# nanoporetech/medaka

Measured on NVIDIA H100. Metric: pileup positions/sec (consensus inference), higher is better.
Workload: dtype f32

## Files before the change

medaka_b200/csrc/gru_wg.cu:

```cuda
#include "common.cuh"
#include "ptx.cuh"
#include "rec_common.cuh"

namespace mdk {

constexpr int RW_THREADS = 256;
constexpr int RW_ABLK = (H / 8) * 64 * 16;
constexpr int RW_XBLK = 2 * 64 * 16;

template <int NT, bool FUSE_X, int OUT>
struct RwCfg {
    static constexpr int N = NT * RT_N;
    static constexpr bool HL = NT == 1;
    static constexpr int ROWS = HL ? 2 * N : N;
    static constexpr int PLANES = HL ? 1 : 2;
    static constexpr int KG = ROWS * 16 + 16;
    static constexpr int HPLANE = (H / 8) * KG;
    static constexpr int XPLANE = 2 * KG;
    static constexpr int HLO = HL ? N * 16 : HPLANE;
    static constexpr int XLO = HL ? N * 16 : XPLANE;
    static constexpr int RED = (RW_THREADS / 32) * NCLS * N;
    static constexpr int wlo_off = 0;
    static constexpr int wxlo_off = wlo_off + 6 * RW_ABLK;
    static constexpr int h_off = wxlo_off + (FUSE_X ? 6 * RW_XBLK : 0);
    static constexpr int x_off = h_off + 2 * PLANES * HPLANE;
    static constexpr int red_off = x_off + (FUSE_X ? 2 * PLANES * XPLANE : 0);
    static constexpr int total = red_off + (OUT == OUT_LOGITS ? 2 * RED * 4 : 0);
    static_assert(total <= 227 * 1024, "smem budget");
};

__device__ __forceinline__ uint32_t ld_u32(const __half *p) { return *reinterpret_cast<const uint32_t *>(p); }

template <int NT, bool FUSE_X, int OUT>
__global__ void __launch_bounds__(RW_THREADS, 1)
rec_tc_kernel(const float *__restrict__ gi, RecX xin, const __half *__restrict__ w_hh, const float *__restrict__ b_hn,
              void *__restrict__ h_out, int64_t B, int64_t T, const float *__restrict__ lin_w,
              float *__restrict__ plog) {
    using L = RwCfg<NT, FUSE_X, OUT>;
    constexpr int N = L::N, NA = N / 2;
    constexpr int NACC = L::ROWS / 2;
    constexpr int NX = FUSE_X ? NACC : NA;
    using MMA = Wgmma<N>;
    using MMA_H = Wgmma<L::ROWS>;
    constexpr bool LOGITS = OUT == OUT_LOGITS;
    extern __shared__ __align__(128) uint8_t smem[];
    const int tid = threadIdx.x, wg = tid >> 7, warp = (tid >> 5) & 3, lane = tid & 31;
    const int gq = lane >> 2, cq = lane & 3;
    const int dir = blockIdx.y;
    const int64_t ntiles = (B + RT_N - 1) / RT_N;
    const int64_t wtile0 = (int64_t)blockIdx.x * NT;
    const int j0 = wg * 64 + warp * 16 + gq;
    const uint32_t sbase = smem_u32(smem);

    for (int i = tid; i < (L::total - L::h_off) / 16; i += RW_THREADS)
        reinterpret_cast<int4 *>(smem + L::h_off)[i] = make_int4(0, 0, 0, 0);
    for (int i = tid; i < 3 * H * (H / 8); i += RW_THREADS) {
        const int kg = i & 15, r = (i >> 4) & (H - 1), gate = i >> 11;
        const uint4 v = *reinterpret_cast<const uint4 *>(w_hh + ((((size_t)dir * 2 + 1) * 3 + gate) * H + r) * H + kg * 8);
        *reinterpret_cast<uint4 *>(smem + L::wlo_off + (gate * 2 + (r >> 6)) * RW_ABLK + kg * 1024 + (r & 63) * 16) = v;
    }
    if (FUSE_X) {
        for (int i = tid; i < 3 * H * 2; i += RW_THREADS) {
            const int kg = i & 1, r = (i >> 1) & (H - 1), gate = i >> 8;
            const uint4 v = *reinterpret_cast<const uint4 *>(xin.w_x + ((((size_t)dir * 2 + 1) * 3 + gate) * H + r) * 16 + kg * 8);
            *reinterpret_cast<uint4 *>(smem + L::wxlo_off + (gate * 2 + (r >> 6)) * RW_XBLK + kg * 1024 + (r & 63) * 16) = v;
        }
    }
    float wlin[2][NCLS];
    if (LOGITS) {
#pragma unroll
        for (int hb = 0; hb < 2; ++hb)
#pragma unroll
            for (int c = 0; c < NCLS; ++c) wlin[hb][c] = lin_w[c * H2 + dir * H + j0 + 8 * hb];
    }
    uint32_t whi[3][H / 16][4];
#pragma unroll
    for (int gate = 0; gate < 3; ++gate)
#pragma unroll
        for (int ks = 0; ks < H / 16; ++ks) {
            const __half *w = w_hh + ((((size_t)dir * 2) * 3 + gate) * H + j0) * H + ks * 16 + 2 * cq;
            whi[gate][ks][0] = ld_u32(w);
            whi[gate][ks][1] = ld_u32(w + 8 * H);
            whi[gate][ks][2] = ld_u32(w + 8);
            whi[gate][ks][3] = ld_u32(w + 8 * H + 8);
        }
    uint32_t wxhi[3][4];
    float bx[3][2] = {};
    if (FUSE_X) {
#pragma unroll
        for (int gate = 0; gate < 3; ++gate) {
            const __half *w = xin.w_x + ((((size_t)dir * 2) * 3 + gate) * H + j0) * 16 + 2 * cq;
            wxhi[gate][0] = ld_u32(w);
            wxhi[gate][1] = ld_u32(w + 8 * 16);
            wxhi[gate][2] = ld_u32(w + 8);
            wxhi[gate][3] = ld_u32(w + 8 * 16 + 8);
            bx[gate][0] = xin.bias[dir * G3 + gate * H + j0];
            bx[gate][1] = xin.bias[dir * G3 + gate * H + j0 + 8];
        }
    }
    const float bhn[2] = {b_hn[dir * H + j0], b_hn[dir * H + j0 + 8]};

    float ar[NACC], az[NACC], an[NACC], axn[NX], hp[NA];
#pragma unroll
    for (int k = 0; k < NA; ++k) hp[k] = 0.f;
    const float *gi_thr = FUSE_X ? nullptr
                                 : gi + wtile0 * T * GI_TS_FLOATS + ((dir * 3 * 4 + (cq >> 1)) * H + j0) * 4 + 2 * (cq & 1);
    auto load_pre = [&](int64_t t) {
#pragma unroll
        for (int i = 0; i < N / 8; ++i)
#pragma unroll
            for (int hb = 0; hb < 2; ++hb) {
                float2 v[3] = {make_float2(0.f, 0.f), make_float2(0.f, 0.f), make_float2(0.f, 0.f)};
                if (FUSE_X) {
#pragma unroll
                    for (int gate = 0; gate < 3; ++gate) v[gate] = make_float2(bx[gate][hb], bx[gate][hb]);
                } else if (i < 2 || wtile0 + (i >> 1) < ntiles) {
                    const float *p = gi_thr + ((i >> 1) * T + t) * GI_TS_FLOATS + (2 * (i & 1) * H + 8 * hb) * 4;
#pragma unroll
                    for (int gate = 0; gate < 3; ++gate) v[gate] = __ldcs(reinterpret_cast<const float2 *>(p + gate * 16 * H));
                }
                const int k = 4 * i + 2 * hb;
                ar[k] = v[0].x; ar[k + 1] = v[0].y;
                az[k] = v[1].x; az[k + 1] = v[1].y;
                axn[k] = v[2].x; axn[k + 1] = v[2].y;
                an[k] = bhn[hb]; an[k + 1] = bhn[hb];
            }
        if constexpr (L::HL) {
#pragma unroll
            for (int k = NA; k < NACC; ++k) {
                ar[k] = 0.f; az[k] = 0.f; an[k] = 0.f;
                if constexpr (FUSE_X) axn[k] = 0.f;
            }
        }
    };
    const int xF = FUSE_X ? xin.F : 1;
    const float *xsrc[NT];
    int xoff[NT];
    float xreg[NT];
#pragma unroll
    for (int m = 0; m < NT; ++m) {
        const int q = tid + RW_THREADS * m, xn = q / xF, xf = q - xn * xF;
        const bool own = FUSE_X && q < N * xF;
        xoff[m] = own ? (xf >> 3) * L::KG + xn * 16 + (xf & 7) * 2 : -1;
        xsrc[m] = (own && wtile0 * RT_N + xn < B) ? xin.feats + ((wtile0 * RT_N + xn) * T) * xF + xf : nullptr;
        xreg[m] = 0.f;
    }
    auto stage_x = [&](int buf, int m, float v) {
        __half hi, lo;
        split_f16(v, hi, lo);
        *reinterpret_cast<__half *>(smem + L::x_off + buf * L::PLANES * L::XPLANE + xoff[m]) = hi;
        *reinterpret_cast<__half *>(smem + L::x_off + buf * L::PLANES * L::XPLANE + L::XLO + xoff[m]) = lo;
    };
    const int64_t t_first = dir ? T - 1 : 0;
    if (FUSE_X) {
#pragma unroll
        for (int m = 0; m < NT; ++m) {
            if (xoff[m] < 0) continue;
            stage_x(0, m, xsrc[m] ? xsrc[m][t_first * xF] : 0.f);
        }
    }
    load_pre(t_first);
    fence_proxy_async_smem();
    __syncthreads();

    constexpr int NW = N / 4;
    auto head_partials = [&](int rb) {
        float v[NW][NCLS];
#pragma unroll
        for (int wl = 0; wl < NW; ++wl) {
            const int k = 4 * (wl >> 1) + (wl & 1);
#pragma unroll
            for (int c = 0; c < NCLS; ++c) v[wl][c] = fmaf(wlin[1][c], hp[k + 2], wlin[0][c] * hp[k]);
        }
        int wbase = 0;
#pragma unroll
        for (int lvl = 0; lvl < 3; ++lvl) {
            const int mask = 16 >> lvl;
            const int half = (NW >> lvl) / 2;
            if (half > 0) {
                const bool up = lane & mask;
#pragma unroll
                for (int w = 0; w < NW / 2; ++w) {
                    if (w >= half) continue;
#pragma unroll
                    for (int c = 0; c < NCLS; ++c) {
                        const float send = up ? v[w][c] : v[w + half][c];
                        const float keep = up ? v[w + half][c] : v[w][c];
                        v[w][c] = keep + __shfl_xor_sync(0xffffffffu, send, mask);
                    }
                }
                if (up) wbase += half;
            } else {
#pragma unroll
                for (int c = 0; c < NCLS; ++c) v[0][c] += __shfl_xor_sync(0xffffffffu, v[0][c], mask);
            }
        }
        if (NW >= 8 || !(lane & 4)) {
            float *red = reinterpret_cast<float *>(smem + L::red_off) + rb * L::RED + (tid >> 5) * NCLS * N;
            const int n = 8 * (wbase >> 1) + 2 * cq + (wbase & 1);
#pragma unroll
            for (int c = 0; c < NCLS; ++c) red[c * N + n] = v[0][c];
        }
    };
    auto head_store = [&](int rb, int64_t t) {
        if (tid >= NCLS * N) return;
        const int c = tid / N, n = tid % N;
        const float *red = reinterpret_cast<const float *>(smem + L::red_off) + rb * L::RED + c * N + n;
        float s = red[0];
#pragma unroll
        for (int w = 1; w < RW_THREADS / 32; ++w) s += red[w * NCLS * N];
        const int64_t wt = wtile0 + n / RT_N;
        if (wt < ntiles) plog[((dir * ntiles + wt) * T + t) * PLOG_TS_FLOATS + c * RT_N + (n & 15)] = s;
    };
    auto store_h0 = [&](int b, int64_t t) {
#pragma unroll
        for (int r = 0; r < NT * 512 / RW_THREADS; ++r) {
            const int q = tid + RW_THREADS * r, row = q & 15, kg = (q >> 4) & 15, p = (q >> 8) & 1, m = q >> 9;
            const int64_t wt = wtile0 + m;
            if (wt >= ntiles) continue;
            const int64_t orow = (wt * T + t) * RT_N + row;
            const int4 v = *reinterpret_cast<const int4 *>(smem + L::h_off + b * L::PLANES * L::HPLANE + p * L::HLO + kg * L::KG +
                                                           (m * RT_N + row) * 16);
            *reinterpret_cast<int4 *>(reinterpret_cast<uint8_t *>(h_out) + (orow >> 7) * (int64_t)XT_TILE_BYTES +
                                      p * XT_PLANE_BYTES + (dir * (H / 8) + kg) * (XT_ROWS * 16) + (orow & (XT_ROWS - 1)) * 16) = v;
        }
    };

#pragma unroll 1
    for (int64_t step = 0; step < T; ++step) {
        const int64_t t = dir ? T - 1 - step : step;
        const int buf = (int)(step & 1);
        const uint32_t hb_addr = sbase + L::h_off + buf * L::PLANES * L::HPLANE;
        wg_fence();
        if constexpr (L::HL) {
#pragma unroll
            for (int ks = 0; ks < H / 16; ++ks) {
                const uint64_t bh = make_smem_desc(hb_addr + ks * 2 * L::KG, L::KG, 128);
#pragma unroll
                for (int gate = 0; gate < 3; ++gate) MMA_H::rs(gate == 0 ? ar : (gate == 1 ? az : an), whi[gate][ks], bh, 1u);
#pragma unroll
                for (int gate = 0; gate < 3; ++gate)
                    MMA::ss(gate == 0 ? ar : (gate == 1 ? az : an),
                            make_smem_desc(sbase + L::wlo_off + (gate * 2 + wg) * RW_ABLK + ks * 2 * 1024, 1024, 128), bh, 1u);
            }
        } else {
#pragma unroll
            for (int gate = 0; gate < 3; ++gate) {
                float(&acc)[NACC] = gate == 0 ? ar : (gate == 1 ? az : an);
#pragma unroll
                for (int ks = 0; ks < H / 16; ++ks) {
                    const uint64_t bh = make_smem_desc(hb_addr + ks * 2 * L::KG, L::KG, 128);
                    MMA::rs(acc, whi[gate][ks], bh, 1u);
                    MMA::rs(acc, whi[gate][ks], make_smem_desc(hb_addr + L::HPLANE + ks * 2 * L::KG, L::KG, 128), 1u);
                    MMA::ss(acc, make_smem_desc(sbase + L::wlo_off + (gate * 2 + wg) * RW_ABLK + ks * 2 * 1024, 1024, 128), bh, 1u);
                }
            }
        }
        if constexpr (FUSE_X) {
            const uint32_t xa = sbase + L::x_off + buf * L::PLANES * L::XPLANE;
            const uint64_t bh = make_smem_desc(xa, L::KG, 128);
            if constexpr (L::HL) {
#pragma unroll
                for (int gate = 0; gate < 3; ++gate) MMA_H::rs(gate == 0 ? ar : (gate == 1 ? az : axn), wxhi[gate], bh, 1u);
#pragma unroll
                for (int gate = 0; gate < 3; ++gate)
                    MMA::ss(gate == 0 ? ar : (gate == 1 ? az : axn),
                            make_smem_desc(sbase + L::wxlo_off + (gate * 2 + wg) * RW_XBLK, 1024, 128), bh, 1u);
            } else {
                const uint64_t bl = make_smem_desc(xa + L::XPLANE, L::KG, 128);
#pragma unroll
                for (int gate = 0; gate < 3; ++gate) {
                    float(&acc)[NACC] = gate == 0 ? ar : (gate == 1 ? az : axn);
                    MMA::rs(acc, wxhi[gate], bh, 1u);
                    MMA::rs(acc, wxhi[gate], bl, 1u);
                    MMA::ss(acc, make_smem_desc(sbase + L::wxlo_off + (gate * 2 + wg) * RW_XBLK, 1024, 128), bh, 1u);
                }
            }
        }
        wg_commit();
        if (FUSE_X && step + 1 < T) {
#pragma unroll
            for (int m = 0; m < NT; ++m)
                if (xsrc[m]) xreg[m] = xsrc[m][(dir ? t - 1 : t + 1) * xF];
        }
        if (OUT == OUT_TILES && step > 0) store_h0(buf, dir ? t + 1 : t - 1);
        if (!FUSE_X && tid == 0 && step + GI_PREFETCH_STEPS < T) {
            const int64_t tp = dir ? t - GI_PREFETCH_STEPS : t + GI_PREFETCH_STEPS;
#pragma unroll
            for (int m = 0; m < NT; ++m) {
                if (wtile0 + m >= ntiles) break;
                const float *blk = gi + ((wtile0 + m) * T + tp) * GI_TS_FLOATS + (int64_t)dir * (GI_TS_FLOATS / 2);
#pragma unroll
                for (int i = 0; i < 12; ++i) bulk_prefetch_l2(blk + i * 512, 2048);
            }
        }
        if (LOGITS && step > 0) {
            if (step > 1) head_store((int)((step - 1) & 1), dir ? t + 2 : t - 2);
            head_partials((int)(step & 1));
        }
        wg_wait_all();
        wg_hold(ar); wg_hold(az); wg_hold(an); wg_hold(axn);

        uint8_t *hw = smem + L::h_off + (buf ^ 1) * L::PLANES * L::HPLANE;
#pragma unroll
        for (int k = 0; k < NA; ++k) {
            float pr = ar[k], pz = az[k], pn = an[k], px = axn[k], r, z;
            if constexpr (L::HL) {
                pr += ar[k + NA]; pz += az[k + NA]; pn += an[k + NA];
                if constexpr (FUSE_X) px += axn[k + NA];
                const float a = 1.f + ex2_approx(fminf(pr, EXP_CLAMP)), b = 1.f + ex2_approx(fminf(pz, EXP_CLAMP));
                const float q = rcp_approx(a * b);
                r = b * q;
                z = a * q;
            } else {
                r = rcp_approx(1.f + ex2_approx(fminf(pr, EXP_CLAMP)));
                z = rcp_approx(1.f + ex2_approx(fminf(pz, EXP_CLAMP)));
            }
            const float en = ex2_approx(fminf(fmaf(r, pn, px), EXP_CLAMP));
            const float n = (en - 1.f) * rcp_approx(en + 1.f);
            hp[k] = fmaf(z, hp[k] - n, n);
            const int j = j0 + 8 * ((k >> 1) & 1), col = 8 * (k >> 2) + 2 * cq + (k & 1);
            __half hi, lo;
            split_f16(hp[k], hi, lo);
            *reinterpret_cast<__half *>(hw + (j >> 3) * L::KG + col * 16 + (j & 7) * 2) = hi;
            *reinterpret_cast<__half *>(hw + L::HLO + (j >> 3) * L::KG + col * 16 + (j & 7) * 2) = lo;
        }
        if (FUSE_X && step + 1 < T) {
#pragma unroll
            for (int m = 0; m < NT; ++m) {
                if (xoff[m] < 0) continue;
                stage_x(buf ^ 1, m, xreg[m]);
            }
        }
        if (OUT == OUT_ROWS) {
#pragma unroll
            for (int k = 0; k < NA; ++k) {
                const int i = k >> 2, n = 8 * i + 2 * cq + (k & 1);
                const int64_t wt = wtile0 + (i >> 1);
                if (wt >= ntiles) continue;
                const int64_t orow = (wt * T + t) * RT_N + (n & 15);
                reinterpret_cast<float *>(h_out)[orow * H2 + dir * H + j0 + 8 * ((k >> 1) & 1)] = hp[k];
            }
        }
        if (FUSE_X || step + 1 < T) load_pre(dir ? t - 1 : t + 1);
        fence_proxy_async_smem();
        __syncthreads();
    }
    if (OUT == OUT_TILES) store_h0((int)(T & 1), dir ? 0 : T - 1);
    if (LOGITS) {
        if (T > 1) head_store((int)((T - 1) & 1), dir ? 1 : T - 2);
        head_partials((int)(T & 1));
        __syncthreads();
        head_store((int)(T & 1), dir ? 0 : T - 1);
    }
}

template <int NT, bool FX, int OUT>
static cudaError_t launch_rec(const float *gi, const RecX &xin, const __half *w_hh_tm, const float *b_hn, void *out,
                              const float *lin_w, int64_t B, int64_t T, cudaStream_t s) {
    auto kern = rec_tc_kernel<NT, FX, OUT>;
    constexpr int smem_bytes = RwCfg<NT, FX, OUT>::total;
    cudaError_t e = cudaFuncSetAttribute(kern, cudaFuncAttributeMaxDynamicSharedMemorySize, smem_bytes);
    if (e != cudaSuccess) return e;
    const int64_t tiles = (B + RT_N - 1) / RT_N;
    dim3 grid((unsigned)((tiles + NT - 1) / NT), NDIR);
    constexpr bool LOGITS = OUT == OUT_LOGITS;
    kern<<<grid, RW_THREADS, smem_bytes, s>>>(gi, xin, w_hh_tm, b_hn, LOGITS ? nullptr : out, B, T, lin_w,
                                              LOGITS ? static_cast<float *>(out) : nullptr);
    return cudaGetLastError();
}

template <int NT>
static cudaError_t launch_rec_nt(const float *gi, const RecX *xin, const __half *w_hh_tm, const float *b_hn, int out_kind,
                                 void *out, const float *lin_w, int64_t B, int64_t T, cudaStream_t s) {
    if (xin)
        return out_kind == OUT_TILES ? launch_rec<NT, true, OUT_TILES>(gi, *xin, w_hh_tm, b_hn, out, nullptr, B, T, s)
                                     : cudaErrorInvalidValue;
    const RecX none{nullptr, nullptr, nullptr, 0};
    switch (out_kind) {
    case OUT_TILES: return launch_rec<NT, false, OUT_TILES>(gi, none, w_hh_tm, b_hn, out, nullptr, B, T, s);
    case OUT_ROWS: return launch_rec<NT, false, OUT_ROWS>(gi, none, w_hh_tm, b_hn, out, nullptr, B, T, s);
    case OUT_LOGITS:
        return lin_w ? launch_rec<NT, false, OUT_LOGITS>(gi, none, w_hh_tm, b_hn, out, lin_w, B, T, s) : cudaErrorInvalidValue;
    }
    return cudaErrorInvalidValue;
}

cudaError_t launch_rec_tc(const float *gi, const RecX *xin, const __half *w_hh_tm, const float *b_hn, int tiles_per_cta,
                          int out_kind, void *out, const float *lin_w, int64_t B, int64_t T, cudaStream_t s) {
    if (B == 0 || T == 0) return cudaSuccess;
    switch (tiles_per_cta) {
    case 1: return launch_rec_nt<1>(gi, xin, w_hh_tm, b_hn, out_kind, out, lin_w, B, T, s);
    case 2: return launch_rec_nt<2>(gi, xin, w_hh_tm, b_hn, out_kind, out, lin_w, B, T, s);
    }
    return cudaErrorInvalidValue;
}

constexpr int GW_THREADS = 256;
constexpr int GW_QK = 8;
constexpr int GW_STAGE_PLANE = GW_QK * XT_ROWS * 16;
constexpr int GW_STAGE = 2 * GW_STAGE_PLANE;
constexpr int GW_NQ = XT_K / 8 / GW_QK;
constexpr int GW_KS = XT_K / 16;
constexpr int GW_TS = XT_ROWS / WT;
constexpr int GW_QUAD = H * 4;
constexpr int GW_QUAD_PAD = GW_QUAD + 16;
constexpr int GW_OUT_OFF = GW_NQ * GW_STAGE;
constexpr int GW_BAR_OFF = GW_OUT_OFF + GW_TS * 4 * GW_QUAD_PAD * 4;
constexpr int GW_SMEM = GW_BAR_OFF + 2 * GW_NQ * 8;
static_assert(GW_SMEM <= 227 * 1024, "smem budget");
static_assert(GW_TS * 4 == 32, "one bulk store per lane of warp 0");

__global__ void __launch_bounds__(GW_THREADS, 1)
gemm_tc_kernel(const uint8_t *__restrict__ x_tiles, const __half *__restrict__ w_in_tm, const float *__restrict__ bias,
               float *__restrict__ gi, int64_t P, int64_t ntiles) {
    extern __shared__ __align__(128) uint8_t smem[];
    uint64_t *full = reinterpret_cast<uint64_t *>(smem + GW_BAR_OFF), *empty = full + GW_NQ;
    float *stg = reinterpret_cast<float *>(smem + GW_OUT_OFF);
    const int tid = threadIdx.x, wg = tid >> 7, warp = (tid >> 5) & 3, lane = tid & 31;
    const int gq = lane >> 2, cq = lane & 3;
    const int blk = blockIdx.x;
    const int j0 = wg * 64 + warp * 16 + gq;
    const uint32_t sbase = smem_u32(smem);
    const int64_t my_tiles = blockIdx.y < ntiles ? (ntiles - 1 - blockIdx.y) / gridDim.y + 1 : 0;
    auto issue = [&](int64_t n, int q) {
        const uint8_t *src = x_tiles + (blockIdx.y + n * gridDim.y) * (int64_t)XT_TILE_BYTES + q * GW_STAGE_PLANE;
        mbar_arrive_expect_tx(&full[q], GW_STAGE);
        bulk_g2s(smem + q * GW_STAGE, src, GW_STAGE_PLANE, &full[q]);
        bulk_g2s(smem + q * GW_STAGE + GW_STAGE_PLANE, src + XT_PLANE_BYTES, GW_STAGE_PLANE, &full[q]);
    };
    if (tid == 0) {
        for (int q = 0; q < GW_NQ; ++q) {
            mbar_init(&full[q], 1);
            mbar_init(&empty[q], GW_THREADS / 32);
        }
        fence_mbar_init();
        if (my_tiles > 0)
            for (int q = 0; q < GW_NQ; ++q) issue(0, q);
    }
    uint32_t wa[2][GW_KS][4];
#pragma unroll
    for (int p = 0; p < 2; ++p)
#pragma unroll
        for (int ks = 0; ks < GW_KS; ++ks) {
            const __half *w = w_in_tm + (((size_t)blk * 2 + p) * H + j0) * H2 + ks * 16 + 2 * cq;
            wa[p][ks][0] = ld_u32(w);
            wa[p][ks][1] = ld_u32(w + 8 * H2);
            wa[p][ks][2] = ld_u32(w + 8);
            wa[p][ks][3] = ld_u32(w + 8 * H2 + 8);
        }
    const float bj[2] = {bias[blk * H + j0], bias[blk * H + j0 + 8]};
    const uint64_t policy = l2_evict_first_policy();
    __syncthreads();
    auto release = [&](int64_t n, int q) {
        if (lane == 0) mbar_arrive(&empty[q]);
        if (tid == 0 && n + 1 < my_tiles) {
            mbar_wait(&empty[q], (uint32_t)(n & 1));
            issue(n + 1, q);
        }
        __syncwarp();
    };
    float acc[64];
#pragma unroll 1
    for (int64_t n = 0; n < my_tiles; ++n) {
#pragma unroll
        for (int q = 0; q < GW_NQ; ++q) {
            mbar_wait(&full[q], (uint32_t)(n & 1));
            wg_fence();
#pragma unroll
            for (int prod = 0; prod < 3; ++prod) {
                const int pa = prod == 2, pb = prod == 1;
#pragma unroll
                for (int kk = 0; kk < GW_QK / 2; ++kk) {
                    const uint64_t b = make_smem_desc(sbase + q * GW_STAGE + pb * GW_STAGE_PLANE + 2 * kk * (XT_ROWS * 16),
                                                      XT_ROWS * 16, 128);
                    Wgmma<128>::rs(acc, wa[pa][q * (GW_QK / 2) + kk], b, (q | prod | kk) ? 1u : 0u);
                }
            }
            wg_commit();
            if (q > 0) {
                wg_wait_1();
                release(n, q - 1);
            }
        }
        wg_wait_all();
        wg_hold(acc);
        release(n, GW_NQ - 1);

        const int64_t tile = blockIdx.y + n * gridDim.y;
        const int64_t prem = P - tile * XT_ROWS;
        if (tid < 32) bulk_wait_read_all();
        __syncthreads();
#pragma unroll
        for (int k = 0; k < 64; k += 2) {
            const int i = k >> 2, hb = (k >> 1) & 1;
            float *o = stg + ((i >> 1) * 4 + 2 * (i & 1) + (cq >> 1)) * GW_QUAD_PAD + (j0 + 8 * hb) * 4 + 2 * (cq & 1);
            *reinterpret_cast<float2 *>(o) = make_float2(acc[k] + bj[hb], acc[k + 1] + bj[hb]);
        }
        fence_proxy_async_smem();
        __syncthreads();
        if (tid < 32) {
            const int ts = lane >> 2, cg = lane & 3;
            if (ts * WT < prem)
                bulk_s2g(gi + (((tile * GW_TS + ts) * 6 + blk) * 4 + cg) * GW_QUAD, stg + lane * GW_QUAD_PAD,
                         GW_QUAD * 4, policy);
            bulk_commit();
        }
    }
    if (tid < 32) bulk_wait_all();
}

cudaError_t launch_gemm_tc(const void *x_tiles, const __half *w_in_tm, const float *bias, float *gi, int64_t P,
                           int sm_count, cudaStream_t s) {
    if (P == 0) return cudaSuccess;
    const int64_t ntiles = (P + XT_ROWS - 1) / XT_ROWS;
    cudaError_t ea = cudaFuncSetAttribute(gemm_tc_kernel, cudaFuncAttributeMaxDynamicSharedMemorySize, GW_SMEM);
    if (ea != cudaSuccess) return ea;
    int64_t ct = sm_count / 6;
    if (ct < 1) ct = 1;
    if (ct > ntiles) ct = ntiles;
    dim3 grid(6, (unsigned)ct);
    gemm_tc_kernel<<<grid, GW_THREADS, GW_SMEM, s>>>(reinterpret_cast<const uint8_t *>(x_tiles), w_in_tm, bias, gi, P, ntiles);
    return cudaGetLastError();
}

__global__ void __launch_bounds__(256, 1)
selftest_kernel(const float *__restrict__ A, const float *__restrict__ Bm, float *__restrict__ D, int N, int K) {
    extern __shared__ __align__(128) uint8_t smem[];
    const int a_plane = 128 * K * 2, b_plane = N * K * 2;
    uint8_t *sa = smem, *sb = smem + 2 * a_plane;
    const int tid = threadIdx.x, wg = tid >> 7, warp = (tid >> 5) & 3, lane = tid & 31;
    for (int i = tid; i < 128 * K; i += 256) {
        const int r = i / K, k = i % K;
        __half hi, lo;
        split_f16(A[i], hi, lo);
        const int off = (k / 8) * (128 * 16) + r * 16 + (k % 8) * 2;
        *reinterpret_cast<__half *>(sa + off) = hi;
        *reinterpret_cast<__half *>(sa + a_plane + off) = lo;
    }
    for (int i = tid; i < N * K; i += 256) {
        const int r = i / K, k = i % K;
        __half hi, lo;
        split_f16(Bm[i], hi, lo);
        const int off = (k / 8) * (N * 16) + r * 16 + (k % 8) * 2;
        *reinterpret_cast<__half *>(sb + off) = hi;
        *reinterpret_cast<__half *>(sb + b_plane + off) = lo;
    }
    fence_proxy_async_smem();
    __syncthreads();
    for (int n0 = 0; n0 < N; n0 += 16) {
        float d[8];
        wg_fence();
        uint32_t acc = 0;
        for (int prod = 0; prod < 3; ++prod) {
            const int pa = (prod == 2), pb = (prod == 1);
            for (int ks = 0; ks < K / 16; ++ks) {
                const uint64_t ad = make_smem_desc(smem_u32(sa + pa * a_plane) + ks * 2 * 128 * 16 + wg * 64 * 16, 128 * 16, 128);
                const uint64_t bd = make_smem_desc(smem_u32(sb + pb * b_plane) + ks * 2 * N * 16 + n0 * 16, N * 16, 128);
                Wgmma<16>::ss(d, ad, bd, acc);
                acc = 1;
            }
        }
        wg_commit();
        wg_wait_all();
        wg_hold(d);
        const int row = wg * 64 + warp * 16 + (lane >> 2);
        for (int k = 0; k < 8; ++k)
            D[(row + 8 * ((k >> 1) & 1)) * N + n0 + 8 * (k >> 2) + 2 * (lane & 3) + (k & 1)] = d[k];
    }
}

int selftest_umma(int device, const float *A, const float *B, float *D, int N, int K, int variant) {
    MDK_REQUIRE(N >= 16 && N <= 128 && N % 16 == 0, MDK_ERR_ARG, "selftest_umma: N must be a multiple of 16 in [16,128]");
    MDK_REQUIRE(K >= 16 && K <= 256 && K % 16 == 0, MDK_ERR_ARG, "selftest_umma: K must be a multiple of 16 in [16,256]");
    MDK_REQUIRE(variant == 0, MDK_ERR_ARG, "selftest_umma: variant must be 0");
    MDK_CUDA(cudaSetDevice(device));
    float *dA = nullptr, *dB = nullptr, *dD = nullptr;
    MDK_CUDA(cudaMalloc(&dA, sizeof(float) * 128 * K));
    MDK_CUDA(cudaMalloc(&dB, sizeof(float) * N * K));
    MDK_CUDA(cudaMalloc(&dD, sizeof(float) * 128 * N));
    MDK_CUDA(cudaMemcpy(dA, A, sizeof(float) * 128 * K, cudaMemcpyHostToDevice));
    MDK_CUDA(cudaMemcpy(dB, B, sizeof(float) * N * K, cudaMemcpyHostToDevice));
    const int smem = 2 * 128 * K * 2 + 2 * N * K * 2;
    MDK_REQUIRE(smem <= 227 * 1024, MDK_ERR_ARG, "selftest_umma: N*K too large for shared memory");
    MDK_CUDA(cudaFuncSetAttribute(selftest_kernel, cudaFuncAttributeMaxDynamicSharedMemorySize, smem));
    selftest_kernel<<<1, 256, smem>>>(dA, dB, dD, N, K);
    MDK_CUDA(cudaGetLastError());
    MDK_CUDA(cudaDeviceSynchronize());
    MDK_CUDA(cudaMemcpy(D, dD, sizeof(float) * 128 * N, cudaMemcpyDeviceToHost));
    cudaFree(dA); cudaFree(dB); cudaFree(dD);
    return MDK_OK;
}

}
```

medaka_b200/csrc/ptx.cuh:

```cuda
#pragma once
#include <cstdint>
#include <cuda_fp16.h>

namespace mdk {

__device__ __forceinline__ uint32_t smem_u32(const void *p) {
    return static_cast<uint32_t>(__cvta_generic_to_shared(p));
}

__device__ __forceinline__ void mbar_init(uint64_t *bar, uint32_t count) {
    asm volatile("mbarrier.init.shared::cta.b64 [%0], %1;" ::"r"(smem_u32(bar)), "r"(count) : "memory");
}
__device__ __forceinline__ void fence_mbar_init() {
    asm volatile("fence.mbarrier_init.release.cluster;" ::: "memory");
}
__device__ __forceinline__ void mbar_arrive_expect_tx(uint64_t *bar, uint32_t bytes) {
    asm volatile("mbarrier.arrive.expect_tx.shared::cta.b64 _, [%0], %1;" ::"r"(smem_u32(bar)), "r"(bytes)
                 : "memory");
}
__device__ __forceinline__ void mbar_arrive(uint64_t *bar) {
    asm volatile("mbarrier.arrive.shared::cta.b64 _, [%0];" ::"r"(smem_u32(bar)) : "memory");
}
__device__ __forceinline__ bool mbar_try_wait(uint64_t *bar, uint32_t parity) {
    uint32_t ok;
    asm volatile(
        "{\n\t.reg .pred p;\n\t"
        "mbarrier.try_wait.parity.shared::cta.b64 p, [%1], %2;\n\t"
        "selp.u32 %0, 1, 0, p;\n\t}"
        : "=r"(ok)
        : "r"(smem_u32(bar)), "r"(parity)
        : "memory");
    return ok != 0;
}
__device__ __forceinline__ void mbar_wait(uint64_t *bar, uint32_t parity) {
    if (mbar_try_wait(bar, parity)) return;
    const long long t0 = clock64();
    while (!mbar_try_wait(bar, parity)) {
        if (clock64() - t0 > 4000000000LL) __trap();
    }
}

__device__ __forceinline__ void fence_proxy_async_smem() {
    asm volatile("fence.proxy.async.shared::cta;" ::: "memory");
}

__device__ __forceinline__ uint32_t cluster_ctarank() {
    uint32_t r;
    asm volatile("mov.u32 %0, %%cluster_ctarank;" : "=r"(r));
    return r;
}
__device__ __forceinline__ uint32_t mapa_shared(uint32_t smem_addr, uint32_t rank) {
    uint32_t r;
    asm volatile("mapa.shared::cluster.u32 %0, %1, %2;" : "=r"(r) : "r"(smem_addr), "r"(rank));
    return r;
}
__device__ __forceinline__ void st_cluster_u32(uint32_t cluster_addr, uint32_t v) {
    asm volatile("st.shared::cluster.u32 [%0], %1;" ::"r"(cluster_addr), "r"(v) : "memory");
}
__device__ __forceinline__ void fence_proxy_async_cluster() {
    asm volatile("fence.proxy.async.shared::cluster;" ::: "memory");
}
__device__ __forceinline__ void mbar_arrive_cluster(uint32_t cluster_addr) {
    asm volatile("mbarrier.arrive.release.cluster.shared::cluster.b64 _, [%0];" ::"r"(cluster_addr) : "memory");
}
__device__ __forceinline__ bool mbar_try_wait_cluster(uint64_t *bar, uint32_t parity) {
    uint32_t ok;
    asm volatile(
        "{\n\t.reg .pred p;\n\t"
        "mbarrier.try_wait.parity.acquire.cluster.shared::cta.b64 p, [%1], %2;\n\t"
        "selp.u32 %0, 1, 0, p;\n\t}"
        : "=r"(ok)
        : "r"(smem_u32(bar)), "r"(parity)
        : "memory");
    return ok != 0;
}
__device__ __forceinline__ void mbar_wait_cluster(uint64_t *bar, uint32_t parity) {
    if (mbar_try_wait_cluster(bar, parity)) return;
    const long long t0 = clock64();
    while (!mbar_try_wait_cluster(bar, parity)) {
        if (clock64() - t0 > 4000000000LL) __trap();
    }
}
__device__ __forceinline__ void cluster_sync_all() {
    asm volatile("barrier.cluster.arrive.release.aligned;\n\tbarrier.cluster.wait.acquire.aligned;" ::: "memory");
}
__device__ __forceinline__ void named_bar_sync(uint32_t id, uint32_t count) {
    asm volatile("bar.sync %0, %1;" ::"r"(id), "r"(count) : "memory");
}

__device__ __forceinline__ void bulk_prefetch_l2(const void *gmem_src, uint32_t bytes) {
    asm volatile("cp.async.bulk.prefetch.L2.global [%0], %1;" ::"l"(gmem_src), "r"(bytes) : "memory");
}

__device__ __forceinline__ void bulk_g2s(void *smem_dst, const void *gmem_src, uint32_t bytes, uint64_t *bar) {
    asm volatile(
        "cp.async.bulk.shared::cluster.global.mbarrier::complete_tx::bytes [%0], [%1], %2, [%3];" ::"r"(
            smem_u32(smem_dst)),
        "l"(gmem_src), "r"(bytes), "r"(smem_u32(bar))
        : "memory");
}
__device__ __forceinline__ uint64_t l2_evict_first_policy() {
    uint64_t p;
    asm volatile("createpolicy.fractional.L2::evict_first.b64 %0, 1.0;" : "=l"(p));
    return p;
}
__device__ __forceinline__ void bulk_s2g(void *gmem_dst, const void *smem_src, uint32_t bytes, uint64_t policy) {
    asm volatile("cp.async.bulk.global.shared::cta.bulk_group.L2::cache_hint [%0], [%1], %2, %3;" ::"l"(gmem_dst),
                 "r"(smem_u32(smem_src)), "r"(bytes), "l"(policy)
                 : "memory");
}
__device__ __forceinline__ void bulk_commit() { asm volatile("cp.async.bulk.commit_group;" ::: "memory"); }
__device__ __forceinline__ void bulk_wait_read_all() { asm volatile("cp.async.bulk.wait_group.read 0;" ::: "memory"); }
__device__ __forceinline__ void bulk_wait_all() { asm volatile("cp.async.bulk.wait_group 0;" ::: "memory"); }

__device__ __forceinline__ uint64_t make_smem_desc(uint32_t smem_addr, uint32_t lbo_bytes, uint32_t sbo_bytes) {
    uint64_t d = 0;
    d |= static_cast<uint64_t>((smem_addr & 0x3FFFF) >> 4);
    d |= static_cast<uint64_t>((lbo_bytes >> 4) & 0x3FFF) << 16;
    d |= static_cast<uint64_t>((sbo_bytes >> 4) & 0x3FFF) << 32;
    return d;
}
__device__ __forceinline__ void wg_fence() { asm volatile("wgmma.fence.sync.aligned;" ::: "memory"); }
__device__ __forceinline__ void wg_commit() { asm volatile("wgmma.commit_group.sync.aligned;" ::: "memory"); }
__device__ __forceinline__ void wg_wait_all() { asm volatile("wgmma.wait_group.sync.aligned 0;" ::: "memory"); }
__device__ __forceinline__ void wg_wait_1() { asm volatile("wgmma.wait_group.sync.aligned 1;" ::: "memory"); }
template <int R>
__device__ __forceinline__ void wg_hold(float (&d)[R]) {
#pragma unroll
    for (int i = 0; i < R; ++i) asm volatile("" : "+f"(d[i])::"memory");
}

template <int N> struct Wgmma;
template <> struct Wgmma<16> {
    __device__ __forceinline__ static void ss(float (&d)[8], uint64_t a, uint64_t b, uint32_t accumulate) {
        asm volatile(
            "{\n\t.reg .pred p;\n\tsetp.ne.b32 p, %10, 0;\n\t"
            "wgmma.mma_async.sync.aligned.m64n16k16.f32.f16.f16 {%0,%1,%2,%3,%4,%5,%6,%7}, %8, %9, p, 1, 1, 0, 0;\n\t}"
            : "+f"(d[0]), "+f"(d[1]), "+f"(d[2]), "+f"(d[3]), "+f"(d[4]), "+f"(d[5]), "+f"(d[6]), "+f"(d[7])
            : "l"(a), "l"(b), "r"(accumulate));
    }
    __device__ __forceinline__ static void rs(float (&d)[8], const uint32_t (&a)[4], uint64_t b, uint32_t accumulate) {
        asm volatile(
            "{\n\t.reg .pred p;\n\tsetp.ne.b32 p, %13, 0;\n\t"
            "wgmma.mma_async.sync.aligned.m64n16k16.f32.f16.f16 {%0,%1,%2,%3,%4,%5,%6,%7}, {%8,%9,%10,%11}, %12, p, 1, 1, 0;\n\t}"
            : "+f"(d[0]), "+f"(d[1]), "+f"(d[2]), "+f"(d[3]), "+f"(d[4]), "+f"(d[5]), "+f"(d[6]), "+f"(d[7])
            : "r"(a[0]), "r"(a[1]), "r"(a[2]), "r"(a[3]), "l"(b), "r"(accumulate));
    }
    __device__ __forceinline__ static void ss(float (&d)[16], uint64_t a, uint64_t b, uint32_t accumulate) {
        asm volatile(
            "{\n\t.reg .pred p;\n\tsetp.ne.b32 p, %10, 0;\n\t"
            "wgmma.mma_async.sync.aligned.m64n16k16.f32.f16.f16 {%0,%1,%2,%3,%4,%5,%6,%7}, %8, %9, p, 1, 1, 0, 0;\n\t}"
            : "+f"(d[0]), "+f"(d[1]), "+f"(d[2]), "+f"(d[3]), "+f"(d[4]), "+f"(d[5]), "+f"(d[6]), "+f"(d[7])
            : "l"(a), "l"(b), "r"(accumulate));
    }
};
template <> struct Wgmma<32> {
    __device__ __forceinline__ static void ss(float (&d)[16], uint64_t a, uint64_t b, uint32_t accumulate) {
        asm volatile(
            "{\n\t.reg .pred p;\n\tsetp.ne.b32 p, %18, 0;\n\t"
            "wgmma.mma_async.sync.aligned.m64n32k16.f32.f16.f16 {%0,%1,%2,%3,%4,%5,%6,%7,%8,%9,%10,%11,%12,%13,%14,%15}, %16, %17, p, 1, 1, 0, 0;\n\t}"
            : "+f"(d[0]), "+f"(d[1]), "+f"(d[2]), "+f"(d[3]), "+f"(d[4]), "+f"(d[5]), "+f"(d[6]), "+f"(d[7]),
              "+f"(d[8]), "+f"(d[9]), "+f"(d[10]), "+f"(d[11]), "+f"(d[12]), "+f"(d[13]), "+f"(d[14]), "+f"(d[15])
            : "l"(a), "l"(b), "r"(accumulate));
    }
    __device__ __forceinline__ static void rs(float (&d)[16], const uint32_t (&a)[4], uint64_t b, uint32_t accumulate) {
        asm volatile(
            "{\n\t.reg .pred p;\n\tsetp.ne.b32 p, %21, 0;\n\t"
            "wgmma.mma_async.sync.aligned.m64n32k16.f32.f16.f16 {%0,%1,%2,%3,%4,%5,%6,%7,%8,%9,%10,%11,%12,%13,%14,%15}, {%16,%17,%18,%19}, %20, p, 1, 1, 0;\n\t}"
            : "+f"(d[0]), "+f"(d[1]), "+f"(d[2]), "+f"(d[3]), "+f"(d[4]), "+f"(d[5]), "+f"(d[6]), "+f"(d[7]),
              "+f"(d[8]), "+f"(d[9]), "+f"(d[10]), "+f"(d[11]), "+f"(d[12]), "+f"(d[13]), "+f"(d[14]), "+f"(d[15])
            : "r"(a[0]), "r"(a[1]), "r"(a[2]), "r"(a[3]), "l"(b), "r"(accumulate));
    }
};
template <> struct Wgmma<128> {
    __device__ __forceinline__ static void ss(float (&d)[64], uint64_t a, uint64_t b, uint32_t accumulate) {
        asm volatile(
            "{\n\t.reg .pred p;\n\tsetp.ne.b32 p, %66, 0;\n\t"
            "wgmma.mma_async.sync.aligned.m64n128k16.f32.f16.f16 {%0,%1,%2,%3,%4,%5,%6,%7,%8,%9,%10,%11,%12,%13,%14,%15,%16,%17,%18,%19,%20,%21,%22,%23,%24,%25,%26,%27,%28,%29,%30,%31,%32,%33,%34,%35,%36,%37,%38,%39,%40,%41,%42,%43,%44,%45,%46,%47,%48,%49,%50,%51,%52,%53,%54,%55,%56,%57,%58,%59,%60,%61,%62,%63}, %64, %65, p, 1, 1, 0, 0;\n\t}"
            : "+f"(d[0]), "+f"(d[1]), "+f"(d[2]), "+f"(d[3]), "+f"(d[4]), "+f"(d[5]), "+f"(d[6]), "+f"(d[7]),
              "+f"(d[8]), "+f"(d[9]), "+f"(d[10]), "+f"(d[11]), "+f"(d[12]), "+f"(d[13]), "+f"(d[14]), "+f"(d[15]),
              "+f"(d[16]), "+f"(d[17]), "+f"(d[18]), "+f"(d[19]), "+f"(d[20]), "+f"(d[21]), "+f"(d[22]), "+f"(d[23]),
              "+f"(d[24]), "+f"(d[25]), "+f"(d[26]), "+f"(d[27]), "+f"(d[28]), "+f"(d[29]), "+f"(d[30]), "+f"(d[31]),
              "+f"(d[32]), "+f"(d[33]), "+f"(d[34]), "+f"(d[35]), "+f"(d[36]), "+f"(d[37]), "+f"(d[38]), "+f"(d[39]),
              "+f"(d[40]), "+f"(d[41]), "+f"(d[42]), "+f"(d[43]), "+f"(d[44]), "+f"(d[45]), "+f"(d[46]), "+f"(d[47]),
              "+f"(d[48]), "+f"(d[49]), "+f"(d[50]), "+f"(d[51]), "+f"(d[52]), "+f"(d[53]), "+f"(d[54]), "+f"(d[55]),
              "+f"(d[56]), "+f"(d[57]), "+f"(d[58]), "+f"(d[59]), "+f"(d[60]), "+f"(d[61]), "+f"(d[62]), "+f"(d[63])
            : "l"(a), "l"(b), "r"(accumulate));
    }
    __device__ __forceinline__ static void rs(float (&d)[64], const uint32_t (&a)[4], uint64_t b, uint32_t accumulate) {
        asm volatile(
            "{\n\t.reg .pred p;\n\tsetp.ne.b32 p, %69, 0;\n\t"
            "wgmma.mma_async.sync.aligned.m64n128k16.f32.f16.f16 {%0,%1,%2,%3,%4,%5,%6,%7,%8,%9,%10,%11,%12,%13,%14,%15,%16,%17,%18,%19,%20,%21,%22,%23,%24,%25,%26,%27,%28,%29,%30,%31,%32,%33,%34,%35,%36,%37,%38,%39,%40,%41,%42,%43,%44,%45,%46,%47,%48,%49,%50,%51,%52,%53,%54,%55,%56,%57,%58,%59,%60,%61,%62,%63}, {%64,%65,%66,%67}, %68, p, 1, 1, 0;\n\t}"
            : "+f"(d[0]), "+f"(d[1]), "+f"(d[2]), "+f"(d[3]), "+f"(d[4]), "+f"(d[5]), "+f"(d[6]), "+f"(d[7]),
              "+f"(d[8]), "+f"(d[9]), "+f"(d[10]), "+f"(d[11]), "+f"(d[12]), "+f"(d[13]), "+f"(d[14]), "+f"(d[15]),
              "+f"(d[16]), "+f"(d[17]), "+f"(d[18]), "+f"(d[19]), "+f"(d[20]), "+f"(d[21]), "+f"(d[22]), "+f"(d[23]),
              "+f"(d[24]), "+f"(d[25]), "+f"(d[26]), "+f"(d[27]), "+f"(d[28]), "+f"(d[29]), "+f"(d[30]), "+f"(d[31]),
              "+f"(d[32]), "+f"(d[33]), "+f"(d[34]), "+f"(d[35]), "+f"(d[36]), "+f"(d[37]), "+f"(d[38]), "+f"(d[39]),
              "+f"(d[40]), "+f"(d[41]), "+f"(d[42]), "+f"(d[43]), "+f"(d[44]), "+f"(d[45]), "+f"(d[46]), "+f"(d[47]),
              "+f"(d[48]), "+f"(d[49]), "+f"(d[50]), "+f"(d[51]), "+f"(d[52]), "+f"(d[53]), "+f"(d[54]), "+f"(d[55]),
              "+f"(d[56]), "+f"(d[57]), "+f"(d[58]), "+f"(d[59]), "+f"(d[60]), "+f"(d[61]), "+f"(d[62]), "+f"(d[63])
            : "r"(a[0]), "r"(a[1]), "r"(a[2]), "r"(a[3]), "l"(b), "r"(accumulate));
    }
};

__host__ __device__ __forceinline__ void split_f16(float v, __half &hi, __half &lo) {
    hi = __float2half_rn(v);
    lo = __float2half_rn(v - __half2float(hi));
}

__device__ __forceinline__ float ldg_stream(const float *p) {
    float v;
    asm volatile("ld.global.nc.L1::no_allocate.f32 %0, [%1];" : "=f"(v) : "l"(p));
    return v;
}

__device__ __forceinline__ float4 ld_stream4(const float *p) {
    float4 v;
    asm volatile("ld.global.nc.L1::no_allocate.v4.f32 {%0,%1,%2,%3}, [%4];"
                 : "=f"(v.x), "=f"(v.y), "=f"(v.z), "=f"(v.w)
                 : "l"(p));
    return v;
}

}
```

Baseline: 178.2 million.

## Split recurrent wgmma into two commit groups to overlap r/z sigmoid with n-gate MMA

In the non-HL (two-plane) path, the fused x-projection MMAs are interleaved per gate, and the async wgmma work is committed in two groups: r and z gates first, then the n gate. After waiting on the first group, the sigmoids for r and z are computed while the n-gate MMAs are still in flight, and the two sigmoids share a single reciprocal. This is meant to hide part of the elementwise latency behind tensor-core work on the sequential critical path. In exchange it adds an extra wait and commit per step, and the reordered MMA issue may change register pressure or pipelining.

```diff
diff --git a/medaka_b200/csrc/gru_wg.cu b/medaka_b200/csrc/gru_wg.cu
--- a/medaka_b200/csrc/gru_wg.cu
+++ b/medaka_b200/csrc/gru_wg.cu
@@ -244,6 +244,7 @@
                             make_smem_desc(sbase + L::wlo_off + (gate * 2 + wg) * RW_ABLK + ks * 2 * 1024, 1024, 128), bh, 1u);
             }
         } else {
+            const uint32_t xa = sbase + L::x_off + buf * L::PLANES * L::XPLANE;
 #pragma unroll
             for (int gate = 0; gate < 3; ++gate) {
                 float(&acc)[NACC] = gate == 0 ? ar : (gate == 1 ? az : an);
@@ -254,30 +255,27 @@
                     MMA::rs(acc, whi[gate][ks], make_smem_desc(hb_addr + L::HPLANE + ks * 2 * L::KG, L::KG, 128), 1u);
                     MMA::ss(acc, make_smem_desc(sbase + L::wlo_off + (gate * 2 + wg) * RW_ABLK + ks * 2 * 1024, 1024, 128), bh, 1u);
                 }
-            }
-        }
-        if constexpr (FUSE_X) {
+                if constexpr (FUSE_X) {
+                    float(&accx)[NACC] = gate == 0 ? ar : (gate == 1 ? az : axn);
+                    const uint64_t bh = make_smem_desc(xa, L::KG, 128);
+                    MMA::rs(accx, wxhi[gate], bh, 1u);
+                    MMA::rs(accx, wxhi[gate], make_smem_desc(xa + L::XPLANE, L::KG, 128), 1u);
+                    MMA::ss(accx, make_smem_desc(sbase + L::wxlo_off + (gate * 2 + wg) * RW_XBLK, 1024, 128), bh, 1u);
+                }
+                if (gate > 0) wg_commit();
+            }
+        }
+        if constexpr (FUSE_X && L::HL) {
             const uint32_t xa = sbase + L::x_off + buf * L::PLANES * L::XPLANE;
             const uint64_t bh = make_smem_desc(xa, L::KG, 128);
-            if constexpr (L::HL) {
-#pragma unroll
-                for (int gate = 0; gate < 3; ++gate) MMA_H::rs(gate == 0 ? ar : (gate == 1 ? az : axn), wxhi[gate], bh, 1u);
-#pragma unroll
-                for (int gate = 0; gate < 3; ++gate)
-                    MMA::ss(gate == 0 ? ar : (gate == 1 ? az : axn),
-                            make_smem_desc(sbase + L::wxlo_off + (gate * 2 + wg) * RW_XBLK, 1024, 128), bh, 1u);
-            } else {
-                const uint64_t bl = make_smem_desc(xa + L::XPLANE, L::KG, 128);
-#pragma unroll
-                for (int gate = 0; gate < 3; ++gate) {
-                    float(&acc)[NACC] = gate == 0 ? ar : (gate == 1 ? az : axn);
-                    MMA::rs(acc, wxhi[gate], bh, 1u);
-                    MMA::rs(acc, wxhi[gate], bl, 1u);
-                    MMA::ss(acc, make_smem_desc(sbase + L::wxlo_off + (gate * 2 + wg) * RW_XBLK, 1024, 128), bh, 1u);
-                }
-            }
-        }
-        wg_commit();
+#pragma unroll
+            for (int gate = 0; gate < 3; ++gate) MMA_H::rs(gate == 0 ? ar : (gate == 1 ? az : axn), wxhi[gate], bh, 1u);
+#pragma unroll
+            for (int gate = 0; gate < 3; ++gate)
+                MMA::ss(gate == 0 ? ar : (gate == 1 ? az : axn),
+                        make_smem_desc(sbase + L::wxlo_off + (gate * 2 + wg) * RW_XBLK, 1024, 128), bh, 1u);
+        }
+        if constexpr (L::HL) wg_commit();
         if (FUSE_X && step + 1 < T) {
 #pragma unroll
             for (int m = 0; m < NT; ++m)
@@ -297,6 +295,17 @@
         if (LOGITS && step > 0) {
             if (step > 1) head_store((int)((step - 1) & 1), dir ? t + 2 : t - 2);
             head_partials((int)(step & 1));
+        }
+        if constexpr (!L::HL) {
+            wg_wait_1();
+            wg_hold(ar); wg_hold(az);
+#pragma unroll
+            for (int k = 0; k < NA; ++k) {
+                const float a = 1.f + ex2_approx(fminf(ar[k], EXP_CLAMP)), b = 1.f + ex2_approx(fminf(az[k], EXP_CLAMP));
+                const float q = rcp_approx(a * b);
+                ar[k] = b * q;
+                az[k] = a * q;
+            }
         }
         wg_wait_all();
         wg_hold(ar); wg_hold(az); wg_hold(an); wg_hold(axn);
@@ -313,8 +322,8 @@
                 r = b * q;
                 z = a * q;
             } else {
-                r = rcp_approx(1.f + ex2_approx(fminf(pr, EXP_CLAMP)));
-                z = rcp_approx(1.f + ex2_approx(fminf(pz, EXP_CLAMP)));
+                r = pr;
+                z = pz;
             }
             const float en = ex2_approx(fminf(fmaf(r, pn, px), EXP_CLAMP));
             const float n = (en - 1.f) * rcp_approx(en + 1.f);
```

New measurement: 180.5 million, median of 6. 1.01x the previous value.

## Write GRU hidden state with stmatrix and interleave gate MMAs per k-slice

Applied to the files above, without the earlier changes.

Replaces the per-element scalar half stores of the hi/lo hidden-state split with packed half2 conversion and stmatrix.x4.trans stores into the shared-memory B operand layout. Reorders the wgmma issue so the three gates are interleaved within each k-slice rather than running a serial chain per gate. Also uses the shared-reciprocal sigmoid trick for the non-HL path. The aim is fewer shared-memory store instructions and more independent MMAs in flight on the recurrent critical path. The risk is an incorrect stmatrix address mapping for the hi/lo planes, which would corrupt the recurrence.

```diff
diff --git a/medaka_b200/csrc/gru_wg.cu b/medaka_b200/csrc/gru_wg.cu
--- a/medaka_b200/csrc/gru_wg.cu
+++ b/medaka_b200/csrc/gru_wg.cu
@@ -15,6 +15,7 @@
     static constexpr int ROWS = HL ? 2 * N : N;
     static constexpr int PLANES = HL ? 1 : 2;
     static constexpr int KG = ROWS * 16 + 16;
+    static_assert(KG % 16 == 0, "stmatrix rows are 16-byte aligned");
     static constexpr int HPLANE = (H / 8) * KG;
     static constexpr int XPLANE = 2 * KG;
     static constexpr int HLO = HL ? N * 16 : HPLANE;
@@ -99,6 +100,8 @@
         }
     }
     const float bhn[2] = {b_hn[dir * H + j0], b_hn[dir * H + j0 + 8]};
+    const uint32_t hst_addr = sbase + L::h_off + (lane >> 4) * L::HLO + (wg * 8 + warp * 2 + ((lane >> 3) & 1)) * L::KG +
+                              (lane & 7) * 16;
 
     float ar[NACC], az[NACC], an[NACC], axn[NX], hp[NA];
 #pragma unroll
@@ -245,15 +248,17 @@
             }
         } else {
 #pragma unroll
-            for (int gate = 0; gate < 3; ++gate) {
-                float(&acc)[NACC] = gate == 0 ? ar : (gate == 1 ? az : an);
-#pragma unroll
-                for (int ks = 0; ks < H / 16; ++ks) {
-                    const uint64_t bh = make_smem_desc(hb_addr + ks * 2 * L::KG, L::KG, 128);
-                    MMA::rs(acc, whi[gate][ks], bh, 1u);
-                    MMA::rs(acc, whi[gate][ks], make_smem_desc(hb_addr + L::HPLANE + ks * 2 * L::KG, L::KG, 128), 1u);
-                    MMA::ss(acc, make_smem_desc(sbase + L::wlo_off + (gate * 2 + wg) * RW_ABLK + ks * 2 * 1024, 1024, 128), bh, 1u);
-                }
+            for (int ks = 0; ks < H / 16; ++ks) {
+                const uint64_t bh = make_smem_desc(hb_addr + ks * 2 * L::KG, L::KG, 128);
+                const uint64_t bl = make_smem_desc(hb_addr + L::HPLANE + ks * 2 * L::KG, L::KG, 128);
+#pragma unroll
+                for (int gate = 0; gate < 3; ++gate) MMA::rs(gate == 0 ? ar : (gate == 1 ? az : an), whi[gate][ks], bh, 1u);
+#pragma unroll
+                for (int gate = 0; gate < 3; ++gate) MMA::rs(gate == 0 ? ar : (gate == 1 ? az : an), whi[gate][ks], bl, 1u);
+#pragma unroll
+                for (int gate = 0; gate < 3; ++gate)
+                    MMA::ss(gate == 0 ? ar : (gate == 1 ? az : an),
+                            make_smem_desc(sbase + L::wlo_off + (gate * 2 + wg) * RW_ABLK + ks * 2 * 1024, 1024, 128), bh, 1u);
             }
         }
         if constexpr (FUSE_X) {
@@ -269,12 +274,13 @@
             } else {
                 const uint64_t bl = make_smem_desc(xa + L::XPLANE, L::KG, 128);
 #pragma unroll
-                for (int gate = 0; gate < 3; ++gate) {
-                    float(&acc)[NACC] = gate == 0 ? ar : (gate == 1 ? az : axn);
-                    MMA::rs(acc, wxhi[gate], bh, 1u);
-                    MMA::rs(acc, wxhi[gate], bl, 1u);
-                    MMA::ss(acc, make_smem_desc(sbase + L::wxlo_off + (gate * 2 + wg) * RW_XBLK, 1024, 128), bh, 1u);
-                }
+                for (int gate = 0; gate < 3; ++gate) MMA::rs(gate == 0 ? ar : (gate == 1 ? az : axn), wxhi[gate], bh, 1u);
+#pragma unroll
+                for (int gate = 0; gate < 3; ++gate) MMA::rs(gate == 0 ? ar : (gate == 1 ? az : axn), wxhi[gate], bl, 1u);
+#pragma unroll
+                for (int gate = 0; gate < 3; ++gate)
+                    MMA::ss(gate == 0 ? ar : (gate == 1 ? az : axn),
+                            make_smem_desc(sbase + L::wxlo_off + (gate * 2 + wg) * RW_XBLK, 1024, 128), bh, 1u);
             }
         }
         wg_commit();
@@ -301,29 +307,26 @@
         wg_wait_all();
         wg_hold(ar); wg_hold(az); wg_hold(an); wg_hold(axn);
 
-        uint8_t *hw = smem + L::h_off + (buf ^ 1) * L::PLANES * L::HPLANE;
 #pragma unroll
         for (int k = 0; k < NA; ++k) {
-            float pr = ar[k], pz = az[k], pn = an[k], px = axn[k], r, z;
+            float pr = ar[k], pz = az[k], pn = an[k], px = axn[k];
             if constexpr (L::HL) {
                 pr += ar[k + NA]; pz += az[k + NA]; pn += an[k + NA];
                 if constexpr (FUSE_X) px += axn[k + NA];
-                const float a = 1.f + ex2_approx(fminf(pr, EXP_CLAMP)), b = 1.f + ex2_approx(fminf(pz, EXP_CLAMP));
-                const float q = rcp_approx(a * b);
-                r = b * q;
-                z = a * q;
-            } else {
-                r = rcp_approx(1.f + ex2_approx(fminf(pr, EXP_CLAMP)));
-                z = rcp_approx(1.f + ex2_approx(fminf(pz, EXP_CLAMP)));
-            }
+            }
+            const float a = 1.f + ex2_approx(fminf(pr, EXP_CLAMP)), b = 1.f + ex2_approx(fminf(pz, EXP_CLAMP));
+            const float q = rcp_approx(a * b);
+            const float r = b * q, z = a * q;
             const float en = ex2_approx(fminf(fmaf(r, pn, px), EXP_CLAMP));
             const float n = (en - 1.f) * rcp_approx(en + 1.f);
             hp[k] = fmaf(z, hp[k] - n, n);
-            const int j = j0 + 8 * ((k >> 1) & 1), col = 8 * (k >> 2) + 2 * cq + (k & 1);
-            __half hi, lo;
-            split_f16(hp[k], hi, lo);
-            *reinterpret_cast<__half *>(hw + (j >> 3) * L::KG + col * 16 + (j & 7) * 2) = hi;
-            *reinterpret_cast<__half *>(hw + L::HLO + (j >> 3) * L::KG + col * 16 + (j & 7) * 2) = lo;
+        }
+#pragma unroll
+        for (int i = 0; i < N / 8; ++i) {
+            uint32_t hi[2], lo[2];
+#pragma unroll
+            for (int hb = 0; hb < 2; ++hb) split_f16x2(hp[4 * i + 2 * hb], hp[4 * i + 2 * hb + 1], hi[hb], lo[hb]);
+            stmatrix_x4_trans(hst_addr + (buf ^ 1) * L::PLANES * L::HPLANE + i * 128, hi[0], hi[1], lo[0], lo[1]);
         }
         if (FUSE_X && step + 1 < T) {
 #pragma unroll
diff --git a/medaka_b200/csrc/ptx.cuh b/medaka_b200/csrc/ptx.cuh
--- a/medaka_b200/csrc/ptx.cuh
+++ b/medaka_b200/csrc/ptx.cuh
@@ -203,9 +203,21 @@
     }
 };
 
+__device__ __forceinline__ void stmatrix_x4_trans(uint32_t smem_addr, uint32_t r0, uint32_t r1, uint32_t r2, uint32_t r3) {
+    asm volatile("stmatrix.sync.aligned.m8n8.x4.trans.shared.b16 [%0], {%1, %2, %3, %4};" ::"r"(smem_addr), "r"(r0),
+                 "r"(r1), "r"(r2), "r"(r3)
+                 : "memory");
+}
+
 __host__ __device__ __forceinline__ void split_f16(float v, __half &hi, __half &lo) {
     hi = __float2half_rn(v);
     lo = __float2half_rn(v - __half2float(hi));
+}
+__device__ __forceinline__ void split_f16x2(float v0, float v1, uint32_t &hi, uint32_t &lo) {
+    const __half2 h = __floats2half2_rn(v0, v1);
+    const __half2 l = __floats2half2_rn(v0 - __low2float(h), v1 - __high2float(h));
+    hi = *reinterpret_cast<const uint32_t *>(&h);
+    lo = *reinterpret_cast<const uint32_t *>(&l);
 }
 
 __device__ __forceinline__ float ldg_stream(const float *p) {
```

Measured after the change: 180.5 million before, 187.5 million after, median of 6. 1.04x the previous value.
